# wen-yuan-zhang/Fast-Learning-NeRF

Hardware: AMD Instinct MI355X
Metric: training rays/sec (Lego-like 800x800, 64+128 samples) + PSNR@N-iters (higher is better)
Workload: dtype f32; 1 GPU; nerf-ours Lego full 800x800 (BASELINE configs[1]), SURVEY 8(d) throughput protocol: 4096 uniformly drawn rays per GPU per step, 64+128 samples, use_viewdirs, white_bkgd, perturb=1, U[0,1) targets, random-init nets, leaf-error table on, fp32-width bf16x6 kernels, plain backward (FASTNERF_COMPACT=0); parallelism=dp1, math_mode=bf16x6, backward=plain (every sample)

## Files before the change

fast-learning-nerf_amd/_lib.py:

```python
import ctypes as C
import os

import torch

HERE = os.path.dirname(os.path.abspath(__file__))
LIB_PATH = os.environ.get('FASTNERF_LIB') or os.path.join(HERE, 'libfastnerf.so')

P = C.c_void_p
I = C.c_int
L = C.c_int64
F = C.c_float
D = C.c_double
U64 = C.c_uint64



class StepArgs(C.Structure):
    _fields_ = (
        [('n', L)] + [(k, P) for k in ('rays_o', 'rays_d', 'target', 't_rand', 'u', 'noise0', 'noise1')]
        + [('seed0', U64), ('seed1', U64), ('leaf_tag', P), ('table', P), ('net_floats', L)]
        + [(k, P) for k in ('params', 'grads', 'adam_m', 'adam_v', 'packed_fwd_c', 'packed_bwd_c', 'packed_fwd_f', 'packed_bwd_f',
                            'rays11', 'z0', 'raw0', 'act0', 'rgb0', 'disp0', 'acc0', 'w0', 'depth0',
                            'z1', 'z_samples', 'z_std', 'raw1', 'act1', 'rgb1', 'disp1', 'acc1', 'w1', 'depth1',
                            'g_rgb', 'g_rgb0', 'loss2', 'draw_ws', 'act_ws', 'dact_ws', 'partial_ws', 'live_ws', 'counts')]
        + [(k, D) for k in ('focal', 'lr', 'beta1', 'beta2', 'eps')]
        + [(k, F) for k in ('near_plane', 'far_plane', 'grad_scale')]
        + [(k, I) for k in ('math_mode', 'N_samples', 'N_importance', 'lindisp', 'perturb', 'white_bkgd', 'ndc', 'H', 'W', 'live',
                            'fwd_flags', 'max_leaves', 'adam_t')]
        + [('occ', P), ('occ_counts', P)])


class OccGrid(C.Structure):
    _fields_ = [('words', P), ('lo', F * 3), ('inv', F * 3), ('n', C.c_int32 * 3), ('outside_occupied', C.c_int32)]


OCC_MAX_LEVELS = 8


class OccCascade(C.Structure):
    _fields_ = [('levels', C.c_int32), ('reserved', C.c_int32), ('level', OccGrid * OCC_MAX_LEVELS)]


STEP_FORWARD, STEP_BWD_FINE, STEP_BWD_COARSE, STEP_UPDATE = 1, 2, 4, 8

SIGNATURES = {
    'fastnerf_version': (I, []),
    'fastnerf_last_error': (C.c_char_p, []),
    'fastnerf_device_cus': (I, []),
    'fastnerf_gen_rays': (I, [I, I, F, F, F, F, P, P, P, P]),
    'fastnerf_gen_rays_pixels': (I, [L, P, P, F, F, F, F, P, P, P]),
    'fastnerf_ndc_rays': (I, [L, I, I, D, F, P, P, P, P, P]),
    'fastnerf_pack_rays': (I, [L, P, P, F, F, I, I, I, D, P, P]),
    'fastnerf_sample_coarse': (I, [L, I, P, I, I, P, U64, P, P]),
    'fastnerf_posenc': (I, [L, I, P, P, P]),
    'fastnerf_mlp_pack': (I, [P, P, P, P]),
    'fastnerf_mlp_fwd': (I, [L, I, P, P, P, P, P, P, P]),
    'fastnerf_mlp_bwd_partial_floats': (L, []),
    'fastnerf_mlp_bwd': (I, [L, I, P, P, P, P, P, P, P, P]),
    'fastnerf_raw2outputs_fwd': (I, [L, I, P, P, P, P, I, P, P, P, P, P, P]),
    'fastnerf_raw2outputs_bwd': (I, [L, I, P, P, P, P, I, P, P, P]),
    'fastnerf_raw2outputs_bwd_full': (I, [L, I, P, P, P, P, I, P, P, P, P, P, P, P, P, P]),
    'fastnerf_sample_pdf_merge': (I, [L, I, I, P, P, I, P, U64, P, P, P, P]),
    'fastnerf_sample_pdf': (I, [L, I, I, P, P, I, P, U64, P, P]),
    'fastnerf_mse_leafmax': (I, [L, P, P, P, F, P, P, P, P, I, P, P]),
    'fastnerf_adam_step': (I, [L, P, P, P, P, D, D, D, D, I, P]),
    'fastnerf_net_floats': (L, [I, I]),
    'fastnerf_mlp_act_floats': (L, [I, L]),
    'fastnerf_mlp_pack_ex': (I, [I, P, P, P, P]),
    'fastnerf_mlp_fwd_ex': (I, [I, L, I, P, P, P, P, P, P, P]),
    'fastnerf_mlp_bwd_ex': (I, [I, L, I, P, P, P, P, P, P, P, P]),
    'fastnerf_mlp_bf16_floats': (L, [I, I, L]),
    'fastnerf_mlp_bf16_partial_floats': (L, []),
    'fastnerf_mlp_bf16_pack': (I, [I, P, P, P, P]),
    'fastnerf_mlp_bf16_fwd': (I, [I, L, I, P, P, P, P, P, P, P]),
    'fastnerf_mlp_bf16_bwd': (I, [I, L, I, P, P, P, P, P, P, P, P]),
    'fastnerf_render_rays_fwd': (I, [I, L, I, I, P, I, I, I, I, P, P, P, P, U64, U64, P, P, P, P] + [P] * 18 + [P]),
    'fastnerf_render_rays_fwd_ex': (I, [I, L, I, I, P, I, I, I, I, P, P, P, P, U64, U64, P, P, P, P] + [P] * 18 + [I, P]),
    'fastnerf_mlp_bf16_fwd_flags': (I, [I, L, I, P, P, P, P, P, I, P]),
    'fastnerf_mlp_fwd_flags_ex': (I, [I, L, I, P, P, P, P, P, I, P]),
    'fastnerf_render_rays_bwd': (I, [I, L, I, I, P, I] + [P] * 20),
    'fastnerf_pp_intersect_sphere': (I, [L, P, P, P, P]),
    'fastnerf_pp_fg_depths': (I, [L, I, F, P, I, P, U64, P, P]),
    'fastnerf_pp_sample_pdf_merge': (I, [L, I, I, P, P, I, P, U64, P, P, P]),
    'fastnerf_pp_perturb_samples': (I, [L, I, P, P, U64, P, P]),
    'fastnerf_pp_sample_pdf': (I, [L, I, I, P, P, I, P, U64, P, P]),
    'fastnerf_pp_depth2pts_outside': (I, [L, I, P, P, P, P, P, P]),
    'fastnerf_pp_composite_fwd': (I, [L, I, I, P, P, P, P, P, P, P, P, P]),
    'fastnerf_pp_composite_bwd': (I, [L, I, I, P, P, P, P, P, P, P, P]),
    'fastnerf_pp_gen_rays': (I, [I, I, P, P, P, P, P]),
    'fastnerf_leaf_sumcount': (I, [L, P, P, P, I, P, P, P]),
    'fastnerf_tree_adjust_mean': (L, [P, P, P, I, D]),
    'fastnerf_tree_create': (P, [I, I, I, I]),
    'fastnerf_tree_destroy': (None, [P]),
    'fastnerf_tree_num_leaves': (I, [P, I]),
    'fastnerf_tree_max_leaves': (I, [P]),
    'fastnerf_tree_min_area': (D, [P, I]),
    'fastnerf_tree_get_leaves': (I, [P, I, P]),
    'fastnerf_tree_set_leaves': (I, [P, I, I, P, D]),
    'fastnerf_tree_leaf_plan': (I, [P, I, D, I, P]),
    'fastnerf_tree_adjust': (L, [P, P, I, D]),
    'fastnerf_tree_epoch_plan': (L, [P, D, I, P, P]),
# ... 99 lines not shown
```

fast-learning-nerf_amd/csrc/mlp_bwd_dw.hip:

```cpp
#include "mlp_common.h"

int fn_launch_dx(int mm, int grid, hipStream_t st, int64_t P, const float* draw, const float* act, const float* params, const float* packed_bwd,
                 float* dact, const NetLayout& L, const int* live_idx, const int* live_cnt);

#define DW_MT 32

template <int WO, int WI, int TO, int TI, bool BIAS, bool RANK1>
__global__ void __launch_bounds__(WO * WI * 64, WO * WI / 4)
mlp_bwd_dw_kernel(int64_t P, const float* __restrict__ dY, int ldy, const float* __restrict__ X, int ldx,
                  const float* __restrict__ draw , float* __restrict__ partial_w,
                  float* __restrict__ partial_b, float* __restrict__ partial_r, const int* __restrict__ live_idx,
                  const int* __restrict__ live_cnt) {
  if (live_idx) P = (int64_t)__builtin_amdgcn_readfirstlane(*live_cnt);
  constexpr int NO = WO * TO * 32, KI = WI * TI * 32;
  constexpr int NTD = WO * WI * 64;
  constexpr int STAGE = DW_MT * (NO + KI) + DW_MT;
  extern __shared__ __attribute__((aligned(16))) float smem[];
  const int tid = threadIdx.x;
  const int lane = tid & 63;
  const int wave = __builtin_amdgcn_readfirstlane(tid >> 6);
  const int wo = wave / WI, wi = wave % WI;
  const int64_t ntile_all = (P + DW_MT - 1) / DW_MT;
  const int64_t per = (ntile_all + gridDim.x - 1) / gridDim.x;
  const int64_t t0 = blockIdx.x * per;
  int64_t t1 = t0 + per;
  if (t1 > ntile_all) t1 = ntile_all;

  f32x16 acc[TO][TI];
#pragma unroll
  for (int a = 0; a < TO; ++a)
#pragma unroll
    for (int b = 0; b < TI; ++b)
#pragma unroll
      for (int r = 0; r < 16; ++r) acc[a][b][r] = 0.f;
  float bsum = 0.f, rsum = 0.f;

  constexpr int YV = (DW_MT * NO / 4 + NTD - 1) / NTD;
  constexpr int XV = (DW_MT * KI / 4 + NTD - 1) / NTD;
  static_assert(DW_MT * NO % 4 == 0 && DW_MT * KI % 4 == 0 && NO <= NTD && KI <= NTD, "stage split");
  float4 ry[YV], rx[XV];
  float rda = 0.f;

  auto load_stage = [&](int64_t t) {
    const int64_t pbase = t * DW_MT;
#pragma unroll
    for (int i = 0; i < YV; ++i) {
      const int e = (i * NTD + tid) * 4;
      const int m = e / NO, c = e % NO;
      const int64_t p = pbase + m;
      ry[i] = (e < DW_MT * NO && p < P) ? *reinterpret_cast<const float4*>(dY + p * ldy + c)
                                        : make_float4(0.f, 0.f, 0.f, 0.f);
    }
#pragma unroll
// ... 294 lines not shown
    const int nwhole = (relmax + 1) / 16;
    int dmain = nwhole >= 5 ? (nwhole - 3) / 2 : 0;
    if (dmain > n2) dmain = n2;
#pragma unroll 1
    for (int d = 0; d < dmain; ++d) pair(d, WHOLE);
#pragma unroll 1
    for (int d = dmain; d < n2; ++d) pair(d, ANY);
  }
  float* pw = partial_w + (int64_t)wg * NO * KI;
#pragma unroll
  for (int i = 0; i < TO; ++i)
#pragma unroll
    for (int j = 0; j < TI; ++j)
#pragma unroll
      for (int r = 0; r < 16; ++r) {
        const int o = (wo * TO + i) * 32 + crow(r, lane);
        const int c = (wi * TI + j) * 32 + (lane & 31);
        pw[(int64_t)o * KI + c] = acc[i][j][r];
      }
  if (BIAS || RANK1) {
#pragma unroll
    for (int k = 0; k < TPW; ++k) {
      const int t = k * NW + wave;
      if (NTILE % NW == 0 || t < NTILE) {
        const float sv = ssum[k] + __shfl_xor(ssum[k], 32, 64);
        if (lane < 32) {
          if (BIAS && t < CTO1) partial_b[(int64_t)wg * NO1 + t * 32 + lane] = sv;
          if (RANK1 && t >= CTO && t < CTO + CTI1) partial_r[(int64_t)wg * KI1 + (t - CTO) * 32 + lane] = sv;
        }
      }
    }
  }
}

template <int WO, int WI, int TO, int TI, bool BIAS, bool RANK1, int CTI2 = 0, int CTO2 = 0>
__global__ void __launch_bounds__(WO * WI * 64, WO * WI / 4)
mlp_bwd_dw6_kernel(int64_t P, const float* __restrict__ dY, const float* __restrict__ X,
                   const float* __restrict__ draw, float* __restrict__ partial_w, float* __restrict__ partial_b,
                   float* __restrict__ partial_r, const int* __restrict__ live_idx, const int* __restrict__ live_cnt,
                   const float* __restrict__ X2 = nullptr, const float* __restrict__ dY2 = nullptr) {
  if (live_idx) P = (int64_t)__builtin_amdgcn_readfirstlane(*live_cnt);
  dw6_body<WO, WI, TO, TI, BIAS, RANK1, CTI2, CTO2>(P, dY, X, draw, partial_w, partial_b, partial_r, live_idx, X2, dY2, (int)blockIdx.x,
                                                    (int)gridDim.x);
}

#define DW_QMAX 256
__host__ __device__ static inline int dw_trunk_chunks(int64_t P, int ncu) {
  const int unit = ncu >= 8 ? ncu / 8 : 1;
  const int64_t nq = (P + 15) / 16;
  int64_t k = (nq + (int64_t)unit * DW_QMAX - 1) / ((int64_t)unit * DW_QMAX);
  k = k < 1 ? 1 : (k > 8 ? 8 : k);
  return unit * (int)k;
}
#define DW_TRUNK_JOBS 7
struct DwTrunk {
  const float* dY[DW_TRUNK_JOBS];
  const float* X[DW_TRUNK_JOBS];
  float* pw[DW_TRUNK_JOBS];
  float* pb[DW_TRUNK_JOBS];
};
__global__ void __launch_bounds__(512, 2)
mlp_bwd_dw6_trunk_kernel(int64_t P, DwTrunk J, const int* __restrict__ live_idx, const int* __restrict__ live_cnt, int ncu) {
  if (live_idx) P = (int64_t)__builtin_amdgcn_readfirstlane(*live_cnt);
  const int nact = dw_trunk_chunks(P, ncu);
  if ((int)blockIdx.x >= nact) return;
  const int job = (int)blockIdx.y;
  dw6_body<4, 2, 2, 4, true, false>(P, J.dY[job], J.X[job], nullptr, J.pw[job], J.pb[job], nullptr, live_idx, nullptr, nullptr,
                                    (int)blockIdx.x, nact);
}

__global__ void __launch_bounds__(128) head_grads_kernel(int64_t P, const float* __restrict__ draw,
                                                          const float* __restrict__ hv,
                                                          float* __restrict__ partial, const int* __restrict__ live_idx,
                                                          const int* __restrict__ live_cnt) {
  const int k = threadIdx.x;
  if (live_idx) P = *live_cnt;
  auto dptr = [&](int64_t q) { return draw + (live_idx ? (int64_t)live_idx[q] : q) * 4; };
  const int64_t per = (P + gridDim.x - 1) / gridDim.x;
  const int64_t pa = blockIdx.x * per;
  int64_t pb = pa + per;
  if (pb > P) pb = P;
  float s0 = 0.f, s1 = 0.f, s2 = 0.f, sb = 0.f;
  int64_t p = pa;
  constexpr int NF = 16;
  for (; p + NF <= pb; p += NF) {
    float4 d[NF];
    float h[NF];
#pragma unroll
    for (int i = 0; i < NF; ++i) {
      d[i] = *reinterpret_cast<const float4*>(dptr(p + i));
      h[i] = hv[(p + i) * 128 + k];
    }
#pragma unroll
    for (int i = 0; i < NF; ++i) {
      s0 = fmaf(d[i].x, h[i], s0); s1 = fmaf(d[i].y, h[i], s1); s2 = fmaf(d[i].z, h[i], s2);
      if (k < 4) sb += (k == 0) ? d[i].x : (k == 1) ? d[i].y : (k == 2) ? d[i].z : d[i].w;
    }
  }
  for (; p < pb; ++p) {
    const float4 d = *reinterpret_cast<const float4*>(dptr(p));
    const float h = hv[p * 128 + k];
    s0 = fmaf(d.x, h, s0); s1 = fmaf(d.y, h, s1); s2 = fmaf(d.z, h, s2);
    if (k < 4) sb += (k == 0) ? d.x : (k == 1) ? d.y : (k == 2) ? d.z : d.w;
  }
  float* o = partial + (int64_t)blockIdx.x * 388;
  o[k] = s0; o[128 + k] = s1; o[256 + k] = s2;
  if (k < 4) o[384 + k] = sb;
}

struct RedSeg {
  int64_t src;
  int64_t wg_stride;
  int64_t dst;
  int nwg, rows, cols, ld, valid_cols;
  int dyn;
  int sc_cols;
  int64_t sc_dst;
};
#define MAX_SEGS 32
struct RedTable {
  RedSeg s[MAX_SEGS];
  int n;
};

__global__ void __launch_bounds__(256) reduce_all_kernel(RedTable tab, const float* __restrict__ partial, float* __restrict__ grads,
                                                          float* __restrict__ scratch, int64_t P, const int* __restrict__ live_cnt, int ncu) {
  RedSeg sg = tab.s[blockIdx.y];
  if (sg.dyn) {
    if (live_cnt) P = (int64_t)*live_cnt;
    const int n = dw_trunk_chunks(P, ncu);
    sg.nwg = n < sg.nwg ? n : sg.nwg;
  }
  const int64_t total = (int64_t)sg.rows * sg.cols;
  const float* src = partial + sg.src;
  for (int64_t e = blockIdx.x * (int64_t)blockDim.x + threadIdx.x; e < total; e += (int64_t)gridDim.x * blockDim.x) {
    const int r = (int)(e / sg.cols), c = (int)(e % sg.cols);
    if (c >= sg.valid_cols) continue;
    constexpr int RS = 16;
    float a[RS];
#pragma unroll
    for (int i = 0; i < RS; ++i) a[i] = 0.f;
    int w = 0;
    for (; w + RS <= sg.nwg; w += RS) {
#pragma unroll
      for (int i = 0; i < RS; ++i) a[i] += src[(int64_t)(w + i) * sg.wg_stride + e];
    }
#pragma unroll
    for (int i = 0; i < RS - 1; ++i)
      if (w + i < sg.nwg) a[i] += src[(int64_t)(w + i) * sg.wg_stride + e];
#pragma unroll
    for (int h = RS / 2; h >= 1; h >>= 1)
#pragma unroll
      for (int i = 0; i < h; ++i) a[i] += a[i + h];
    if (c < sg.sc_cols) scratch[sg.sc_dst + (int64_t)r * sg.sc_cols + c] = a[0];
    else grads[sg.dst + (int64_t)r * sg.ld + c] = a[0];
  }
}

__global__ void __launch_bounds__(256) unfold_kernel(const float* __restrict__ G, const float* __restrict__ params, float* __restrict__ grads,
                                                      int64_t VW, int64_t VB, int64_t FW, int64_t FB) {
  __shared__ double As[16][17], Bs[16][17];
  const int tx = threadIdx.x & 15, ty = threadIdx.x >> 4;
  const int b = blockIdx.x;
  if (b == 384) {
    const int i = threadIdx.x;
    double s = 0.0;
    for (int o = 0; o < 128; ++o) s = fma((double)params[VW + (int64_t)o * 283 + i], (double)grads[VB + o], s);
    grads[FB + i] = (float)s;
    return;
  }
  const bool wf = b < 256;
  const int r0 = wf ? (b >> 4) * 16 : ((b - 256) >> 4) * 16, c0 = (b & 15) * 16;
  const int K = wf ? 128 : 256;
  double s = 0.0;
  for (int k0 = 0; k0 < K; k0 += 16) {
    if (wf) {
// ... 37 lines not shown
  }
  return o;
}
extern "C" int64_t fastnerf_mlp_bwd_partial_floats(void) {
  return dw_job_base(12, num_cus(), 96) + (int64_t)HEAD_MAX_WG * 388;
}

template <int WO, int WI, int TO, int TI, bool BIAS, bool RANK1, int MM = MM_F32, int CTI2 = 0, int CTO2 = 0>
static int launch_dw(int64_t P, const float* dY, int ldy, const float* X, int ldx, const float* draw, float* base,
                     int nwg, hipStream_t st, const int* live_idx = nullptr, const int* live_cnt = nullptr,
                     const float* X2 = nullptr, const float* dY2 = nullptr, float* pr_at = nullptr) {
  constexpr int NO = WO * TO * 32, KI = WI * TI * 32;
  float* pw = base;
  float* pb = base + (int64_t)nwg * NO * KI;
  float* pr = pr_at ? pr_at : pb + (BIAS ? (int64_t)nwg * (NO - CTO2 * 32) : 0);
  if constexpr (MM == MM_X6) {
    if (ldy != NO - CTO2 * 32 || ldx != KI - CTI2 * 32 || (CTI2 > 0) != (X2 != nullptr) || (CTO2 > 0) != (dY2 != nullptr)) {
      fn::set_error("launch_dw: the bf16x6 dW kernel needs ld == width (and X2 / dY2 exactly when CTI2 / CTO2 > 0)");
      return -1;
    }
    constexpr int lds6 = 2 * (WO * TO + WI * TI) * 3 * 1024 + 128;
    auto kern6 = mlp_bwd_dw6_kernel<WO, WI, TO, TI, BIAS, RANK1, CTI2, CTO2>;
    static bool attr6 = false;
    if (!attr6) {
      FN_HIP(hipFuncSetAttribute(reinterpret_cast<const void*>(kern6), hipFuncAttributeMaxDynamicSharedMemorySize, lds6));
      attr6 = true;
    }
    hipLaunchKernelGGL(kern6, dim3(nwg), dim3(WO * WI * 64), lds6, st, P, dY, X, draw, pw, pb, pr, live_idx, live_cnt, X2, dY2);
    FN_LAUNCH_CHECK();
    return 0;
  } else {
    static_assert(MM == MM_F32 && CTI2 == 0 && CTO2 == 0, "two-tensor jobs exist for the bf16x6 dW kernel only");
    constexpr int STAGE = DW_MT * (NO + KI) + DW_MT;
    const size_t lds = 2 * STAGE * sizeof(float);
    auto kern = mlp_bwd_dw_kernel<WO, WI, TO, TI, BIAS, RANK1>;
    static bool attr = false;
    if (!attr) {
      FN_HIP(hipFuncSetAttribute(reinterpret_cast<const void*>(kern), hipFuncAttributeMaxDynamicSharedMemorySize, (int)lds));
      attr = true;
    }
    hipLaunchKernelGGL(kern, dim3(nwg), dim3(WO * WI * 64), lds, st, P, dY, ldy, X, ldx, draw, pw, pb, pr, live_idx, live_cnt);
    FN_LAUNCH_CHECK();
    return 0;
  }
}

static void add_seg(RedTable& T, int64_t src, int64_t wg_stride, int nwg, int rows, int cols, int64_t dst, int ld,
                    int valid_cols, int dyn = 0, int sc_cols = 0, int64_t sc_dst = 0) {
  RedSeg& s = T.s[T.n++];
  s.src = src; s.wg_stride = wg_stride; s.nwg = nwg; s.rows = rows; s.cols = cols; s.dst = dst; s.ld = ld;
  s.valid_cols = valid_cols; s.dyn = dyn; s.sc_cols = sc_cols; s.sc_dst = sc_dst;
}

template <int MM>
static int bwd_launch_t(int kind, int64_t n, int S, const float* draw, const float* act, const float* params,
                      const float* packed_bwd, float* dact, float* partial, float* grads, const int* live_idx,
                      const int* live_cnt, fn_stream_t stream) {
  constexpr int MW = MM;
  const NetLayout& L = layout_of(kind);
  const int PEP = L.pe_pad;
  hipStream_t st = fn::S(stream);
  const int64_t P = n * S;
  const int64_t ntiles = (P + TM - 1) / TM;
  const int ncu = num_cus();
  int grid = ncu * WG_PER_CU;
  if (ntiles < grid) grid = (int)ntiles;
  if (int rc_dx = fn_launch_dx(MM, grid, st, P, draw, act, params, packed_bwd, dact, L, live_idx, live_cnt)) return rc_dx;

  const int nwg = ncu;
  RedTable T;
  T.n = 0;
  int rc;
  const float* a_pe = act + act_pe(P, PEP);
  auto region = [&](int j) { return partial + dw_job_base(j, ncu, PEP); };
  auto segs = [&](int j, int64_t dstW, int ld, int validc, int64_t dstB, int64_t dstR, int dyn = 0) {
    const DwJobDesc d = dw_job(j, PEP);
    const int64_t b = dw_job_base(j, ncu, PEP);
    add_seg(T, b, (int64_t)d.NO * d.KI, nwg, d.NO, d.KI, dstW, ld, validc, dyn);
    int64_t o = b + (int64_t)nwg * d.NO * d.KI;
    if (d.bias) { add_seg(T, o, d.NO, nwg, 1, d.NO, dstB, d.NO, d.NO, dyn); o += (int64_t)nwg * d.NO; }
    if (d.rank1) add_seg(T, o, d.KI, nwg, 1, d.KI, dstR, d.KI, d.KI, dyn);
  };
  if constexpr (MW == MM_X6) {
    if (PEP == 64) rc = launch_dw<8, 2, 2, 1, true, false, MW, 0, 8>(P, dact + dact_y(P, 0), 256, a_pe, 64, nullptr, region(0), nwg, st, live_idx, live_cnt, nullptr, dact + dact_y(P, 5));
    else rc = launch_dw<8, 1, 2, 3, true, false, MW, 0, 8>(P, dact + dact_y(P, 0), 256, a_pe, 96, nullptr, region(0), nwg, st, live_idx, live_cnt, nullptr, dact + dact_y(P, 5));
    if (rc) return rc;
    const int64_t b0 = dw_job_base(0, ncu, PEP);
    add_seg(T, b0, (int64_t)512 * PEP, nwg, 256, PEP, L.LW[0], L.in_pe, L.in_pe);
    add_seg(T, b0 + (int64_t)256 * PEP, (int64_t)512 * PEP, nwg, 256, PEP, L.LW[5], 256 + L.in_pe, L.in_pe);
    add_seg(T, b0 + (int64_t)nwg * 512 * PEP, 256, nwg, 1, 256, L.LB[0], 256, 256);
  } else {
    if (PEP == 64) rc = launch_dw<4, 1, 2, 2, true, false, MW>(P, dact + dact_y(P, 0), 256, a_pe, 64, nullptr, region(0), nwg, st, live_idx, live_cnt);
    else rc = launch_dw<4, 1, 2, 3, true, false, MW>(P, dact + dact_y(P, 0), 256, a_pe, 96, nullptr, region(0), nwg, st, live_idx, live_cnt);
    if (rc) return rc;
    segs(0, L.LW[0], L.in_pe, L.in_pe, L.LB[0], 0);
  }
  if constexpr (MW != MM_X6) {
    for (int l = 1; l < 8; ++l) {
      if ((rc = launch_dw<4, 2, 2, 4, true, false, MW>(P, dact + dact_y(P, l), 256, act + act_h(P, PEP, l - 1), 256, nullptr, region(l), nwg, st, live_idx, live_cnt))) return rc;
      segs(l, L.LW[l] + (l == 5 ? L.in_pe : 0), l == 5 ? 256 + L.in_pe : 256, 256, L.LB[l], 0);
    }
  }
  if constexpr (MW != MM_X6) {
    if (PEP == 64) rc = launch_dw<4, 1, 2, 2, false, false, MW>(P, dact + dact_y(P, 5), 256, a_pe, 64, nullptr, region(8), nwg, st, live_idx, live_cnt);
    else rc = launch_dw<4, 1, 2, 3, false, false, MW>(P, dact + dact_y(P, 5), 256, a_pe, 96, nullptr, region(8), nwg, st, live_idx, live_cnt);
    if (rc) return rc;
    segs(8, L.LW[5], 256 + L.in_pe, L.in_pe, 0, 0);
  }
  if constexpr (MW == MM_X6) {
    DwTrunk J;
    for (int l = 1; l < 8; ++l) {
      J.dY[l - 1] = dact + dact_y(P, l);
      J.X[l - 1] = act + act_h(P, PEP, l - 1);
      J.pw[l - 1] = region(l);
      J.pb[l - 1] = region(l) + (int64_t)nwg * 256 * 256;
    }
    constexpr int lds6 = 2 * 16 * 3 * 1024 + 128;
    static bool attr_t = false;
    if (!attr_t) {
      FN_HIP(hipFuncSetAttribute(reinterpret_cast<const void*>(mlp_bwd_dw6_trunk_kernel), hipFuncAttributeMaxDynamicSharedMemorySize, lds6));
      attr_t = true;
    }
    hipLaunchKernelGGL(mlp_bwd_dw6_trunk_kernel, dim3(dw_trunk_chunks(P, ncu), DW_TRUNK_JOBS), dim3(512), lds6, st, P, J, live_idx, live_cnt, ncu);
    FN_LAUNCH_CHECK();
    for (int l = 1; l < 8; ++l) segs(l, L.LW[l] + (l == 5 ? L.in_pe : 0), l == 5 ? 256 + L.in_pe : 256, 256, L.LB[l], 0, 1);
  }
  float* const pr_view = region(9);
  const int64_t g_off = dw_job_base(9, ncu, PEP) + (int64_t)nwg * 256;
  if constexpr (MW == MM_X6) {
    if ((rc = launch_dw<4, 3, 1, 3, true, true, MW, 1, 0>(P, dact + dact_yv(P), 128, act + act_h(P, PEP, 7), 256, draw, region(10), nwg, st,
                                                    live_idx, live_cnt, act + act_vpe(P, PEP), nullptr, pr_view))) return rc;
    const int64_t b10 = dw_job_base(10, ncu, PEP);
    add_seg(T, b10, 128 * 288, nwg, 128, 288, L.VW, 283, 283, 0, 256, g_off);
    add_seg(T, b10 + (int64_t)nwg * 128 * 288, 128, nwg, 1, 128, L.VB, 128, 128);
  } else {
    if ((rc = launch_dw<2, 4, 2, 2, true, true, MW>(P, dact + dact_yv(P), 128, act + act_h(P, PEP, 7), 256, draw, region(10), nwg, st, live_idx, live_cnt,
                                              nullptr, nullptr, pr_view))) return rc;
    const int64_t b10 = dw_job_base(10, ncu, PEP);
    add_seg(T, b10, 128 * 256, nwg, 128, 256, L.VW, 283, 256, 0, 256, g_off);
    add_seg(T, b10 + (int64_t)nwg * 128 * 256, 128, nwg, 1, 128, L.VB, 128, 128);
    if ((rc = launch_dw<4, 1, 1, 1, false, false, MW>(P, dact + dact_yv(P), 128, act + act_vpe(P, PEP), 32, nullptr, region(11), nwg, st, live_idx, live_cnt))) return rc;
    segs(11, L.VW + 256, 283, 27, 0, 0);
  }
  add_seg(T, dw_job_base(9, ncu, PEP), 256, nwg, 1, 256, L.AW, 256, 256);
  {
    const int hg = HEAD_MAX_WG;
    const int64_t hb = dw_job_base(12, ncu, PEP);
    hipLaunchKernelGGL(head_grads_kernel, dim3(hg), dim3(128), 0, st, P, draw, act + act_hv(P, PEP), partial + hb, live_idx, live_cnt);
    FN_LAUNCH_CHECK();
    add_seg(T, hb, 388, hg, 1, 388, L.RW, 388, 387);
    add_seg(T, hb + 387, 388, hg, 1, 1, L.AB, 1, 1);
  }
  hipLaunchKernelGGL(reduce_all_kernel, dim3(256, T.n), dim3(256), 0, st, T, partial, grads, partial, P, live_cnt, ncu);
  FN_LAUNCH_CHECK();
  hipLaunchKernelGGL(unfold_kernel, dim3(385), dim3(256), 0, st, partial + g_off, params, grads, L.VW, L.VB, L.FW, L.FB);
  FN_LAUNCH_CHECK();
  return 0;
}
static int bwd_launch(int kind, int64_t n, int S, const float* draw, const float* act, const float* params,
                      const float* packed_bwd, float* dact, float* partial, float* grads, const int* live_idx,
                      const int* live_cnt, fn_stream_t stream, int mm = MM_F32) {
  return mm == MM_X6 ? bwd_launch_t<MM_X6>(kind, n, S, draw, act, params, packed_bwd, dact, partial, grads, live_idx, live_cnt, stream)
                     : bwd_launch_t<MM_F32>(kind, n, S, draw, act, params, packed_bwd, dact, partial, grads, live_idx, live_cnt, stream);
}
extern "C" int fastnerf_mlp_bwd_ex(int kind, int64_t n, int S, const float* draw, const float* act,
                                   const float* params, const float* packed_bwd, float* dact, float* partial,
                                   float* grads, fn_stream_t stream) {
  FN_CHECK_ARG(kind >= 0 && kind <= 2 && n > 0 && S >= 1, "kind in 0..2, n>0, S>=1");
  FN_CHECK_ARG(draw && act && params && packed_bwd && dact && partial && grads, "null pointer");
  return bwd_launch(kind, n, S, draw, act, params, packed_bwd, dact, partial, grads, nullptr, nullptr, stream);
}
extern "C" int fastnerf_mlp_bwd_live_ex(int kind, int64_t n, int S, const float* draw, const float* act,
                                        const float* params, const float* packed_bwd, float* dact, float* partial,
                                        float* grads, const int32_t* live_idx, const int32_t* live_cnt,
                                        fn_stream_t stream) {
  FN_CHECK_ARG(kind >= 0 && kind <= 2 && n > 0 && S >= 1, "kind in 0..2, n>0, S>=1");
  FN_CHECK_ARG(draw && act && params && packed_bwd && dact && partial && grads && live_idx && live_cnt, "null pointer");
  return bwd_launch(kind, n, S, draw, act, params, packed_bwd, dact, partial, grads, live_idx, live_cnt, stream);
}
extern "C" int fastnerf_mlp_bwd(int64_t n, int S, const float* draw, const float* act, const float* params,
                                const float* packed_bwd, float* dact, float* partial, float* grads,
                                fn_stream_t stream) {
  return fastnerf_mlp_bwd_ex(0, n, S, draw, act, params, packed_bwd, dact, partial, grads, stream);
}

extern "C" int fastnerf_mlp_x6_bwd(int kind, int64_t n, int S, const float* draw, const float* act, const float* params,
                                   const float* packed_bwd, float* dact, float* partial, float* grads, fn_stream_t stream) {
  FN_CHECK_ARG(kind >= 0 && kind <= 2 && n > 0 && S >= 1, "kind in 0..2, n>0, S>=1");
  FN_CHECK_ARG(draw && act && params && packed_bwd && dact && partial && grads, "null pointer");
  return bwd_launch(kind, n, S, draw, act, params, packed_bwd, dact, partial, grads, nullptr, nullptr, stream, MM_X6);
}
extern "C" int fastnerf_mlp_x6_bwd_live(int kind, int64_t n, int S, const float* draw, const float* act, const float* params,
                                        const float* packed_bwd, float* dact, float* partial, float* grads,
                                        const int32_t* live_idx, const int32_t* live_cnt, fn_stream_t stream) {
  FN_CHECK_ARG(kind >= 0 && kind <= 2 && n > 0 && S >= 1, "kind in 0..2, n>0, S>=1");
  FN_CHECK_ARG(draw && act && params && packed_bwd && dact && partial && grads && live_idx && live_cnt, "null pointer");
  return bwd_launch(kind, n, S, draw, act, params, packed_bwd, dact, partial, grads, live_idx, live_cnt, stream, MM_X6);
}
```

fast-learning-nerf_amd/csrc/render.cpp:

```cpp
#include <stdint.h>
#include "../../include/fastnerf.h"

namespace fn {
void set_error(const char* fmt, ...);
const char* occ_cascade_fault(const fn_occ_cascade* c);
}

struct MlpMode {
  int (*pack)(int kind, const float* params, float* packed_fwd, float* packed_bwd, fn_stream_t);
  int (*fwd)(int kind, int64_t n, int S, const float* rays11, const float* z, const float* params, const float* packed_fwd, float* raw,
             float* act, int flags, fn_stream_t);
  int (*fwd_list)(int kind, int64_t n, int S, const float* rays11, const float* z, const float* params, const float* packed_fwd,
                  float* raw, const int32_t* live_idx, const int32_t* live_cnt, int flags, fn_stream_t);
  int (*fwd_live)(int kind, int64_t n, int S, const float* rays11, const float* z, const float* params, const float* packed_fwd,
                  float* act, const int32_t* live_idx, const int32_t* live_cnt, fn_stream_t);
  int (*bwd)(int kind, int64_t n, int S, const float* draw, const float* act, const float* params, const float* packed_bwd, float* dact,
             float* partial, float* grads, fn_stream_t);
  int (*bwd_live)(int kind, int64_t n, int S, const float* draw, const float* act, const float* params, const float* packed_bwd,
                  float* dact, float* partial, float* grads, const int32_t* live_idx, const int32_t* live_cnt, fn_stream_t);
};

static int fwd_fp32(int kind, int64_t n, int S, const float* rays11, const float* z, const float* params, const float* packed_fwd,
                    float* raw, float* act, int flags, fn_stream_t stream) {
  return act ? fastnerf_mlp_fwd_ex(kind, n, S, rays11, z, params, packed_fwd, raw, act, stream)
             : fastnerf_mlp_fwd_flags_ex(kind, n, S, rays11, z, params, packed_fwd, raw, flags, stream);
}

static int fwd_bf16(int kind, int64_t n, int S, const float* rays11, const float* z, const float* params, const float* packed_fwd,
                    float* raw, float* act, int flags, fn_stream_t stream) {
  return act ? fastnerf_mlp_bf16_fwd(kind, n, S, rays11, z, params, packed_fwd, raw, act, stream)
             : fastnerf_mlp_bf16_fwd_flags(kind, n, S, rays11, z, params, packed_fwd, raw, flags, stream);
}

static const MlpMode modes[3] = {
    {fastnerf_mlp_pack_ex, fwd_fp32, fastnerf_mlp_fwd_list_ex, fastnerf_mlp_fwd_live_ex, fastnerf_mlp_bwd_ex, fastnerf_mlp_bwd_live_ex},
    {fastnerf_mlp_bf16_pack, fwd_bf16, fastnerf_mlp_bf16_fwd_list, fastnerf_mlp_bf16_fwd_live, fastnerf_mlp_bf16_bwd,
     fastnerf_mlp_bf16_bwd_live},
    {fastnerf_mlp_x6_pack, fastnerf_mlp_x6_fwd, fastnerf_mlp_x6_fwd_list, fastnerf_mlp_x6_fwd_live, fastnerf_mlp_x6_bwd,
     fastnerf_mlp_x6_bwd_live},
};

struct RrFwd {
  const char* fname;
  int math_mode;
  int64_t n;
  int N_samples, N_importance;
  const float* rays11;
  int lindisp, perturb, det, white_bkgd;
  const float *t_rand, *u, *noise0, *noise1;
  uint64_t seed0, seed1;
  const float *params_c, *packed_c, *params_f, *packed_f;
  float *z0, *raw0, *rgb0, *disp0, *acc0, *w0, *depth0, *z1, *z_samples, *z_std, *raw1, *rgb1, *disp1, *acc1, *w1, *depth1;
  int flags;
  fn_stream_t stream;
};

static bool rr_fwd_scalars(const RrFwd& a) {
  if (a.math_mode < 0 || a.math_mode > 2 || a.n < 0 || a.N_samples < 2 || a.N_importance < 0) {
// ... 101 lines not shown
                                                    int lindisp, int perturb, int det, int white_bkgd, const float* t_rand,
                                                    const float* u, uint64_t seed0, uint64_t seed1, const float* params_c,
                                                    const float* packed_c, const float* params_f, const float* packed_f,
                                                    const fn_occ_cascade* cascade, int32_t* live_ws, int32_t* counts_out, float* z0,
                                                    float* raw0, float* rgb0, float* disp0, float* acc0, float* w0, float* depth0,
                                                    float* z1, float* z_samples, float* z_std, float* raw1, float* rgb1, float* disp1,
                                                    float* acc1, float* w1, float* depth1, int flags, fn_stream_t stream) {
  return rr_fwd_occ({"fastnerf_render_rays_fwd_occ_cascade", math_mode, n, N_samples, N_importance, rays11, lindisp, perturb, det,
                     white_bkgd, t_rand, u, nullptr, nullptr, seed0, seed1, params_c, packed_c, params_f, packed_f, z0, raw0, rgb0,
                     disp0, acc0, w0, depth0, z1, z_samples, z_std, raw1, rgb1, disp1, acc1, w1, depth1, flags, stream},
                    nullptr, cascade, live_ws, counts_out);
}

extern "C" int fastnerf_render_rays_fwd(int math_mode, int64_t n, int N_samples, int N_importance, const float* rays11,
                                        int lindisp, int perturb, int det, int white_bkgd, const float* t_rand, const float* u,
                                        const float* noise0, const float* noise1, uint64_t seed0, uint64_t seed1,
                                        const float* params_c, const float* packed_c, const float* params_f,
                                        const float* packed_f, float* z0, float* raw0, float* act0, float* rgb0,
                                        float* disp0, float* acc0, float* w0, float* depth0, float* z1,
                                        float* z_samples, float* z_std, float* raw1, float* act1, float* rgb1,
                                        float* disp1, float* acc1, float* w1, float* depth1, fn_stream_t stream) {
  return fastnerf_render_rays_fwd_ex(math_mode, n, N_samples, N_importance, rays11, lindisp, perturb, det, white_bkgd, t_rand, u,
                                     noise0, noise1, seed0, seed1, params_c, packed_c, params_f, packed_f, z0, raw0, act0, rgb0,
                                     disp0, acc0, w0, depth0, z1, z_samples, z_std, raw1, act1, rgb1, disp1, acc1, w1, depth1, 0,
                                     stream);
}

static int rr_bwd(int math_mode, int64_t n, int N_samples, int N_importance, const float* rays11,
                  int white_bkgd, const float* g_rgb, const float* g_rgb0, const float* noise0,
                  const float* noise1, const float* z0, const float* raw0, const float* act0,
                  const float* z1, const float* raw1, const float* act1, const float* params_c,
                  const float* packed_bwd_c, const float* params_f, const float* packed_bwd_f,
                  float* draw_ws, float* dact_ws, float* partial_ws, float* grads_c, float* grads_f,
                  int passes, fn_stream_t stream) {
  if (math_mode < 0 || math_mode > 2 || n <= 0 || N_samples < 2 || N_importance < 0) {
    fn::set_error("fastnerf_render_rays_bwd: bad argument: math_mode in {0,1,2}, n>0, N_samples>=2, N_importance>=0");
    return -1;
  }
  if (!rays11 || !z0 || !raw0 || !act0 || !params_c || !packed_bwd_c || !draw_ws || !dact_ws || !partial_ws || !grads_c) {
    fn::set_error("fastnerf_render_rays_bwd: null pointer (coarse pass)");
    return -1;
  }
  int rc;
  auto mlp = [&](int S, const float* act, const float* params, const float* packed, float* grads) {
    return modes[math_mode].bwd(0, n, S, draw_ws, act, params, packed, dact_ws, partial_ws, grads, stream);
  };
  const float* g_coarse = g_rgb;
  if (N_importance > 0) {
    if (!g_rgb || !g_rgb0 || !z1 || !raw1 || !act1 || !params_f || !packed_bwd_f || !grads_f) {
      fn::set_error("fastnerf_render_rays_bwd: null pointer (fine pass)");
      return -1;
    }
    const int S1 = N_samples + N_importance;
    if (passes & 1) {
      if ((rc = fastnerf_raw2outputs_bwd(n, S1, raw1, z1, rays11, noise1, white_bkgd, g_rgb, draw_ws, stream))) return rc;
      if ((rc = mlp(S1, act1, params_f, packed_bwd_f, grads_f))) return rc;
    }
    g_coarse = g_rgb0;
  }
  if (!g_coarse) {
    fn::set_error("fastnerf_render_rays_bwd: null gradient");
    return -1;
  }
  if (!(passes & 2)) return 0;
  if ((rc = fastnerf_raw2outputs_bwd(n, N_samples, raw0, z0, rays11, noise0, white_bkgd, g_coarse, draw_ws, stream))) return rc;
  return mlp(N_samples, act0, params_c, packed_bwd_c, grads_c);
}

extern "C" int fastnerf_render_rays_bwd(int math_mode, int64_t n, int N_samples, int N_importance, const float* rays11,
                                        int white_bkgd, const float* g_rgb, const float* g_rgb0, const float* noise0,
                                        const float* noise1, const float* z0, const float* raw0, const float* act0,
                                        const float* z1, const float* raw1, const float* act1, const float* params_c,
                                        const float* packed_bwd_c, const float* params_f, const float* packed_bwd_f,
                                        float* draw_ws, float* dact_ws, float* partial_ws, float* grads_c, float* grads_f,
                                        fn_stream_t stream) {
  return rr_bwd(math_mode, n, N_samples, N_importance, rays11, white_bkgd, g_rgb, g_rgb0, noise0, noise1, z0, raw0, act0, z1, raw1,
                act1, params_c, packed_bwd_c, params_f, packed_bwd_f, draw_ws, dact_ws, partial_ws, grads_c, grads_f, 3, stream);
}


static int rr_bwd_live(int math_mode, int64_t n, int N_samples, int N_importance, const float* rays11, int white_bkgd,
                       const float* g_rgb, const float* g_rgb0, const float* noise0, const float* noise1,
                       const float* z0, const float* raw0, const float* z1, const float* raw1,
                       const float* params_c, const float* packed_fwd_c, const float* packed_bwd_c,
                       const float* params_f, const float* packed_fwd_f, const float* packed_bwd_f,
                       float* draw_ws, float* act_ws, float* dact_ws, float* partial_ws, int32_t* live_ws,
                       float* grads_c, float* grads_f, int32_t* counts_out, int passes, fn_stream_t stream) {
  if (math_mode < 0 || math_mode > 2 || n <= 0 || N_samples < 2 || N_importance < 0) {
    fn::set_error("fastnerf_render_rays_bwd_live: bad argument: math_mode in {0,1,2}, n>0, N_samples>=2, N_importance>=0");
    return -1;
  }
  if (!rays11 || !z0 || !raw0 || !params_c || !packed_fwd_c || !packed_bwd_c || !draw_ws || !act_ws || !dact_ws ||
      !partial_ws || !live_ws || !grads_c) {
    fn::set_error("fastnerf_render_rays_bwd_live: null pointer (coarse pass)");
    return -1;
  }
  const int S1 = N_samples + N_importance;
  int32_t* cnt = live_ws;
  int32_t* idx = live_ws + 4;
  int32_t* cws = idx + n * (int64_t)S1;
  int rc;
  auto pass = [&](int S, const float* z, const float* raw, const float* noise, const float* g, const float* params,
                  const float* pf, const float* pb, float* grads, int32_t* cnt_out) -> int {
    if ((rc = fastnerf_raw2outputs_bwd(n, S, raw, z, rays11, noise, white_bkgd, g, draw_ws, stream))) return rc;
    if ((rc = fastnerf_compact_live(n * (int64_t)S, draw_ws, idx, cnt_out, cws, stream))) return rc;
    if ((rc = modes[math_mode].fwd_live(0, n, S, rays11, z, params, pf, act_ws, idx, cnt_out, stream))) return rc;
// ... 123 lines not shown
```

include/fastnerf.h:

```cpp
#ifndef FASTNERF_H
#define FASTNERF_H
#include <stdint.h>
#ifdef __cplusplus
extern "C" {
#endif

typedef void* fn_stream_t;

int fastnerf_version(void);
const char* fastnerf_last_error(void);
int fastnerf_device_cus(void);

int fastnerf_gen_rays(int H, int W, float fx, float fy, float cx, float cy, const float* c2w_host,
                      float* rays_o, float* rays_d, fn_stream_t stream);
int fastnerf_gen_rays_pixels(int64_t n, const int32_t* pix, const float* poses, float fx, float fy, float cx,
                             float cy, float* rays_o, float* rays_d, fn_stream_t stream);
int fastnerf_ndc_rays(int64_t n, int H, int W, double focal, float near, const float* rays_o, const float* rays_d,
                      float* out_o, float* out_d, fn_stream_t stream);
int fastnerf_pack_rays(int64_t n, const float* rays_o, const float* rays_d, float near, float far, int ndc, int H,
                       int W, double focal, float* rays11, fn_stream_t stream);
int fastnerf_sample_coarse(int64_t n, int S, const float* rays11, int lindisp, int perturb, const float* t_rand,
                           uint64_t seed, float* z, fn_stream_t stream);
int fastnerf_posenc(int64_t n, int L, const float* x, float* out, fn_stream_t stream);

#define FASTNERF_NET_PARAMS 595844
#define FASTNERF_PACKED_FWD 593920
#define FASTNERF_PACKED_BWD 557056
#define FASTNERF_ACT_FLOATS 2592
#define FASTNERF_ACT_SLACK 8192
#define FASTNERF_DACT_FLOATS 2432

int fastnerf_mlp_pack(const float* params, float* packed_fwd, float* packed_bwd, fn_stream_t stream);
int fastnerf_mlp_fwd(int64_t n, int S, const float* rays11, const float* z, const float* params,
                     const float* packed_fwd, float* raw, float* act, fn_stream_t stream);
int64_t fastnerf_mlp_bwd_partial_floats(void);
int fastnerf_mlp_bwd(int64_t n, int S, const float* draw, const float* act, const float* params,
                     const float* packed_bwd, float* dact, float* partial, float* grads, fn_stream_t stream);

int fastnerf_raw2outputs_fwd(int64_t n, int S, const float* raw, const float* z, const float* rays11,
                             const float* noise, int white_bkgd, float* rgb_map, float* disp, float* acc,
                             float* weights, float* depth, fn_stream_t stream);
int fastnerf_raw2outputs_bwd(int64_t n, int S, const float* raw, const float* z, const float* rays11,
                             const float* noise, int white_bkgd, const float* g_rgb, float* draw,
                             fn_stream_t stream);
int fastnerf_raw2outputs_bwd_full(int64_t n, int S, const float* raw, const float* z, const float* rays11,
                                  const float* noise, int white_bkgd, const float* acc, const float* depth,
                                  const float* g_rgb, const float* g_disp, const float* g_acc, const float* g_w,
                                  const float* g_depth, float* draw, fn_stream_t stream);
int fastnerf_sample_pdf_merge(int64_t n, int S, int Ni, const float* z, const float* weights, int det,
                              const float* u, uint64_t seed, float* z_out, float* z_samples, float* z_std,
                              fn_stream_t stream);

int fastnerf_sample_pdf(int64_t n, int M, int Ni, const float* bins, const float* weights, int det, const float* u,
                        uint64_t seed, float* samples, fn_stream_t stream);

int fastnerf_mse_leafmax(int64_t n, const float* rgb, const float* rgb0, const float* target, float grad_scale,
                         float* g_rgb, float* g_rgb0, float* loss2, const int32_t* leaf_tag, int max_leaves,
                         uint32_t* table, fn_stream_t stream);
int fastnerf_adam_step(int64_t n, float* params, const float* grads, float* m, float* v, double lr, double beta1,
                       double beta2, double eps, int step, fn_stream_t stream);

int64_t fastnerf_net_floats(int kind, int what);
int64_t fastnerf_mlp_act_floats(int kind, int64_t n_points);
int fastnerf_mlp_pack_ex(int kind, const float* params, float* packed_fwd, float* packed_bwd, fn_stream_t stream);
// ... 252 lines not shown
```

Baseline: 245,500 rays/s.

## Merge fine and coarse bf16x6 trunk weight-gradient passes into one paired launch

In bf16x6 mode with both passes requested, the fine and coarse backward passes now defer their trunk weight-gradient kernel and reductions. A single paired kernel then covers both networks' trunk jobs in one grid, followed by the two reductions. The coarse pass runs on a separately allocated side workspace (dact and partial buffers), so the two passes do not overwrite each other. This is meant to fill the GPU better, since each trunk launch alone may underuse the CUs, and to remove a launch boundary. In exchange it costs extra device memory and a lazy hipMalloc, and it falls back to the old path when allocation fails or during graph capture.

```diff
diff --git a/fast-learning-nerf_amd/_lib.py b/fast-learning-nerf_amd/_lib.py
--- a/fast-learning-nerf_amd/_lib.py
+++ b/fast-learning-nerf_amd/_lib.py
@@ -47,6 +47,7 @@
     'fastnerf_version': (I, []),
     'fastnerf_last_error': (C.c_char_p, []),
     'fastnerf_device_cus': (I, []),
+    'fastnerf_x6_pair_launches': (L, []),
     'fastnerf_gen_rays': (I, [I, I, F, F, F, F, P, P, P, P]),
     'fastnerf_gen_rays_pixels': (I, [L, P, P, F, F, F, F, P, P, P]),
     'fastnerf_ndc_rays': (I, [L, I, I, D, F, P, P, P, P, P]),
diff --git a/fast-learning-nerf_amd/csrc/dw_pair.h b/fast-learning-nerf_amd/csrc/dw_pair.h
--- /dev/null
+++ b/fast-learning-nerf_amd/csrc/dw_pair.h
@@ -0,0 +1,34 @@
+#pragma once
+#include <stdint.h>
+
+#define DW_TRUNK_JOBS 7
+struct DwTrunk {
+  const float* dY[DW_TRUNK_JOBS];
+  const float* X[DW_TRUNK_JOBS];
+  float* pw[DW_TRUNK_JOBS];
+  float* pb[DW_TRUNK_JOBS];
+};
+
+struct RedSeg {
+  int64_t src;
+  int64_t wg_stride;
+  int64_t dst;
+  int nwg, rows, cols, ld, valid_cols;
+  int dyn;
+  int sc_cols;
+  int64_t sc_dst;
+};
+#define MAX_SEGS 32
+struct RedTable {
+  RedSeg s[MAX_SEGS];
+  int n;
+};
+
+struct DwDeferred {
+  DwTrunk J;
+  RedTable T;
+  int64_t P, g_off;
+  const float* params;
+  float *partial, *grads;
+  int kind;
+};
diff --git a/fast-learning-nerf_amd/csrc/mlp_bwd_dw.hip b/fast-learning-nerf_amd/csrc/mlp_bwd_dw.hip
--- a/fast-learning-nerf_amd/csrc/mlp_bwd_dw.hip
+++ b/fast-learning-nerf_amd/csrc/mlp_bwd_dw.hip
@@ -1,4 +1,8 @@
 #include "mlp_common.h"
+#include "dw_pair.h"
+#include <atomic>
+#include <map>
+#include <utility>
 
 int fn_launch_dx(int mm, int grid, hipStream_t st, int64_t P, const float* draw, const float* act, const float* params, const float* packed_bwd,
                  float* dact, const NetLayout& L, const int* live_idx, const int* live_cnt);
@@ -399,13 +403,6 @@
   k = k < 1 ? 1 : (k > 8 ? 8 : k);
   return unit * (int)k;
 }
-#define DW_TRUNK_JOBS 7
-struct DwTrunk {
-  const float* dY[DW_TRUNK_JOBS];
-  const float* X[DW_TRUNK_JOBS];
-  float* pw[DW_TRUNK_JOBS];
-  float* pb[DW_TRUNK_JOBS];
-};
 __global__ void __launch_bounds__(512, 2)
 mlp_bwd_dw6_trunk_kernel(int64_t P, DwTrunk J, const int* __restrict__ live_idx, const int* __restrict__ live_cnt, int ncu) {
   if (live_idx) P = (int64_t)__builtin_amdgcn_readfirstlane(*live_cnt);
@@ -414,6 +411,25 @@
   const int job = (int)blockIdx.y;
   dw6_body<4, 2, 2, 4, true, false>(P, J.dY[job], J.X[job], nullptr, J.pw[job], J.pb[job], nullptr, live_idx, nullptr, nullptr,
                                     (int)blockIdx.x, nact);
+}
+
+struct DwTrunkPair {
+  DwTrunk J[2];
+  int64_t P[2];
+};
+__global__ void __launch_bounds__(512, 2)
+mlp_bwd_dw6_trunk_pair_kernel(DwTrunkPair A, int ncu) {
+  const int c0 = dw_trunk_chunks(A.P[0], ncu);
+  int b = (int)blockIdx.x;
+  const int pass = b >= DW_TRUNK_JOBS * c0 ? 1 : 0;
+  if (pass) b -= DW_TRUNK_JOBS * c0;
+  const int64_t P = A.P[pass];
+  const int nact = pass ? dw_trunk_chunks(P, ncu) : c0;
+  const int job = b / nact;
+  if (job >= DW_TRUNK_JOBS) return;
+  const DwTrunk& J = A.J[pass];
+  dw6_body<4, 2, 2, 4, true, false>(P, J.dY[job], J.X[job], nullptr, J.pw[job], J.pb[job], nullptr, nullptr, nullptr, nullptr, b - job * nact,
+                                    nact);
 }
 
 __global__ void __launch_bounds__(128) head_grads_kernel(int64_t P, const float* __restrict__ draw,
@@ -455,20 +471,6 @@
   if (k < 4) o[384 + k] = sb;
 }
 
-struct RedSeg {
-  int64_t src;
-  int64_t wg_stride;
-  int64_t dst;
-  int nwg, rows, cols, ld, valid_cols;
-  int dyn;
-  int sc_cols;
-  int64_t sc_dst;
-};
-#define MAX_SEGS 32
-struct RedTable {
-  RedSeg s[MAX_SEGS];
-  int n;
-};
 
 __global__ void __launch_bounds__(256) reduce_all_kernel(RedTable tab, const float* __restrict__ partial, float* __restrict__ grads,
                                                           float* __restrict__ scratch, int64_t P, const int* __restrict__ live_cnt, int ncu) {
@@ -612,10 +614,40 @@
   s.valid_cols = valid_cols; s.dyn = dyn; s.sc_cols = sc_cols; s.sc_dst = sc_dst;
 }
 
+#define FN_MAX_DEV 64
+template <class K>
+static int trunk_lds_attr(K kern, bool (&done)[FN_MAX_DEV], int lds) {
+  int dev = 0;
+  FN_HIP(hipGetDevice(&dev));
+  if (dev < 0 || dev >= FN_MAX_DEV || !done[dev]) {
+    FN_HIP(hipFuncSetAttribute(reinterpret_cast<const void*>(kern), hipFuncAttributeMaxDynamicSharedMemorySize, lds));
+    if (dev >= 0 && dev < FN_MAX_DEV) done[dev] = true;
+  }
+  return 0;
+}
+constexpr int DW_TRUNK_LDS = 2 * 16 * 3 * 1024 + 128;
+static int trunk_chunks_fit(int64_t P, int ncu, int nwg) {
+  if (dw_trunk_chunks(P, ncu) > nwg) {
+    fn::set_error("mlp_bwd: the trunk launch needs %d chunks per job, the partial regions hold %d (a device with fewer than 8 CUs?)",
+                  dw_trunk_chunks(P, ncu), nwg);
+    return -1;
+  }
+  return 0;
+}
+
+static int bwd_reduce(const RedTable& T, const NetLayout& L, int64_t P, const float* params, float* partial, float* grads, int64_t g_off,
+                      const int* live_cnt, int ncu, hipStream_t st) {
+  hipLaunchKernelGGL(reduce_all_kernel, dim3(256, T.n), dim3(256), 0, st, T, partial, grads, partial, P, live_cnt, ncu);
+  FN_LAUNCH_CHECK();
+  hipLaunchKernelGGL(unfold_kernel, dim3(385), dim3(256), 0, st, partial + g_off, params, grads, L.VW, L.VB, L.FW, L.FB);
+  FN_LAUNCH_CHECK();
+  return 0;
+}
+
 template <int MM>
 static int bwd_launch_t(int kind, int64_t n, int S, const float* draw, const float* act, const float* params,
                       const float* packed_bwd, float* dact, float* partial, float* grads, const int* live_idx,
-                      const int* live_cnt, fn_stream_t stream) {
+                      const int* live_cnt, fn_stream_t stream, DwDeferred* defer = nullptr) {
   constexpr int MW = MM;
   const NetLayout& L = layout_of(kind);
   const int PEP = L.pe_pad;
@@ -675,14 +707,15 @@
       J.pw[l - 1] = region(l);
       J.pb[l - 1] = region(l) + (int64_t)nwg * 256 * 256;
     }
-    constexpr int lds6 = 2 * 16 * 3 * 1024 + 128;
-    static bool attr_t = false;
-    if (!attr_t) {
-      FN_HIP(hipFuncSetAttribute(reinterpret_cast<const void*>(mlp_bwd_dw6_trunk_kernel), hipFuncAttributeMaxDynamicSharedMemorySize, lds6));
-      attr_t = true;
-    }
-    hipLaunchKernelGGL(mlp_bwd_dw6_trunk_kernel, dim3(dw_trunk_chunks(P, ncu), DW_TRUNK_JOBS), dim3(512), lds6, st, P, J, live_idx, live_cnt, ncu);
-    FN_LAUNCH_CHECK();
+    if ((rc = trunk_chunks_fit(P, ncu, nwg))) return rc;
+    if (defer) {
+      defer->J = J;
+    } else {
+      static bool attr_t[FN_MAX_DEV] = {};
+      if ((rc = trunk_lds_attr(mlp_bwd_dw6_trunk_kernel, attr_t, DW_TRUNK_LDS))) return rc;
+      hipLaunchKernelGGL(mlp_bwd_dw6_trunk_kernel, dim3(dw_trunk_chunks(P, ncu), DW_TRUNK_JOBS), dim3(512), DW_TRUNK_LDS, st, P, J, live_idx, live_cnt, ncu);
+      FN_LAUNCH_CHECK();
+    }
     for (int l = 1; l < 8; ++l) segs(l, L.LW[l] + (l == 5 ? L.in_pe : 0), l == 5 ? 256 + L.in_pe : 256, 256, L.LB[l], 0, 1);
   }
   float* const pr_view = region(9);
@@ -711,12 +744,95 @@
     add_seg(T, hb, 388, hg, 1, 388, L.RW, 388, 387);
     add_seg(T, hb + 387, 388, hg, 1, 1, L.AB, 1, 1);
   }
-  hipLaunchKernelGGL(reduce_all_kernel, dim3(256, T.n), dim3(256), 0, st, T, partial, grads, partial, P, live_cnt, ncu);
+  if (defer) {
+    defer->T = T; defer->P = P; defer->g_off = g_off; defer->params = params; defer->partial = partial; defer->grads = grads; defer->kind = kind;
+    return 0;
+  }
+  return bwd_reduce(T, L, P, params, partial, grads, g_off, live_cnt, ncu, st);
+}
+
+namespace fn {
+struct PairWs {
+  float *dact = nullptr, *partial = nullptr;
+  int64_t dact_cap = 0, partial_cap = 0;
+  int64_t refused = 0;
+};
+static std::mutex g_pair_mu;
+static std::map<std::pair<int, hipStream_t>, PairWs> g_pair;
+static std::atomic<int64_t> g_pair_launches{0};
+
+static bool pair_grow(PairWs& w, float*& p, int64_t& cap, int64_t need) {
+  if (cap >= need) return true;
+  if (w.refused > 0 && need >= w.refused) return false;
+  hipStreamCaptureMode mode = hipStreamCaptureModeRelaxed;
+  (void)hipThreadExchangeStreamCaptureMode(&mode);
+  if (p) (void)hipFree(p);
+  p = nullptr;
+  cap = 0;
+  const bool ok = hipMalloc(reinterpret_cast<void**>(&p), sizeof(float) * (size_t)need) == hipSuccess;
+  (void)hipThreadExchangeStreamCaptureMode(&mode);
+  if (!ok) {
+    (void)hipGetLastError();
+    p = nullptr;
+    w.refused = need;
+    fprintf(stderr, "fastnerf: no memory for the side workspace of the paired bf16x6 backward (%.2f GB): this stream keeps the per-pass trunk launches\n",
+            4e-9 * (double)need);
+    return false;
+  }
+  cap = need;
+  return true;
+}
+
+bool x6_pair_workspace(int64_t P_coarse, fn_stream_t stream, float** dact2, float** partial2) {
+  hipStream_t st = S(stream);
+  hipStreamCaptureStatus cs = hipStreamCaptureStatusNone;
+  if (hipStreamIsCapturing(st, &cs) != hipSuccess) {
+    (void)hipGetLastError();
+    return false;
+  }
+  if (cs != hipStreamCaptureStatusNone) return false;
+  int dev = 0;
+  if (hipGetDevice(&dev) != hipSuccess) return false;
+  std::lock_guard<std::mutex> lk(g_pair_mu);
+  PairWs& w = g_pair[{dev, st}];
+  if (!pair_grow(w, w.dact, w.dact_cap, P_coarse * (int64_t)DACT_FLOATS) ||
+      !pair_grow(w, w.partial, w.partial_cap, fastnerf_mlp_bwd_partial_floats()))
+    return false;
+  *dact2 = w.dact;
+  *partial2 = w.partial;
+  return true;
+}
+
+int x6_pair_pass(DwDeferred* d, int64_t n, int S, const float* draw, const float* act, const float* params, const float* packed_bwd,
+                 float* dact, float* partial, float* grads, fn_stream_t stream) {
+  FN_CHECK_ARG(d && n > 0 && S >= 1, "d != NULL, n>0, S>=1");
+  FN_CHECK_ARG(draw && act && params && packed_bwd && dact && partial && grads, "null pointer");
+  return bwd_launch_t<MM_X6>(0, n, S, draw, act, params, packed_bwd, dact, partial, grads, nullptr, nullptr, stream, d);
+}
+
+int x6_pair_finish(const DwDeferred* fine, const DwDeferred* coarse, fn_stream_t stream) {
+  hipStream_t st = S(stream);
+  const int ncu = num_cus();
+  const DwDeferred* d[2] = {fine, coarse};
+  DwTrunkPair A;
+  int nwg = 0;
+  for (int k = 0; k < 2; ++k) {
+    A.J[k] = d[k]->J;
+    A.P[k] = d[k]->P;
+    nwg += DW_TRUNK_JOBS * dw_trunk_chunks(A.P[k], ncu);
+  }
+  static bool attr_p[FN_MAX_DEV] = {};
+  if (int rc = trunk_lds_attr(mlp_bwd_dw6_trunk_pair_kernel, attr_p, DW_TRUNK_LDS)) return rc;
+  hipLaunchKernelGGL(mlp_bwd_dw6_trunk_pair_kernel, dim3(nwg), dim3(512), DW_TRUNK_LDS, st, A, ncu);
   FN_LAUNCH_CHECK();
-  hipLaunchKernelGGL(unfold_kernel, dim3(385), dim3(256), 0, st, partial + g_off, params, grads, L.VW, L.VB, L.FW, L.FB);
-  FN_LAUNCH_CHECK();
+  g_pair_launches.fetch_add(1, std::memory_order_relaxed);
+  for (int k = 0; k < 2; ++k)
+    if (int rc = bwd_reduce(d[k]->T, layout_of(d[k]->kind), d[k]->P, d[k]->params, d[k]->partial, d[k]->grads, d[k]->g_off, nullptr, ncu, st)) return rc;
   return 0;
 }
+}
+extern "C" int64_t fastnerf_x6_pair_launches(void) { return fn::g_pair_launches.load(std::memory_order_relaxed); }
+
 static int bwd_launch(int kind, int64_t n, int S, const float* draw, const float* act, const float* params,
                       const float* packed_bwd, float* dact, float* partial, float* grads, const int* live_idx,
                       const int* live_cnt, fn_stream_t stream, int mm = MM_F32) {
diff --git a/fast-learning-nerf_amd/csrc/render.cpp b/fast-learning-nerf_amd/csrc/render.cpp
--- a/fast-learning-nerf_amd/csrc/render.cpp
+++ b/fast-learning-nerf_amd/csrc/render.cpp
@@ -1,9 +1,14 @@
 #include <stdint.h>
 #include "../../include/fastnerf.h"
+#include "dw_pair.h"
 
 namespace fn {
 void set_error(const char* fmt, ...);
 const char* occ_cascade_fault(const fn_occ_cascade* c);
+bool x6_pair_workspace(int64_t P_coarse, fn_stream_t stream, float** dact2, float** partial2);
+int x6_pair_pass(DwDeferred* d, int64_t n, int S, const float* draw, const float* act, const float* params, const float* packed_bwd,
+                 float* dact, float* partial, float* grads, fn_stream_t stream);
+int x6_pair_finish(const DwDeferred* fine, const DwDeferred* coarse, fn_stream_t stream);
 }
 
 struct MlpMode {
@@ -211,6 +216,15 @@
       return -1;
     }
     const int S1 = N_samples + N_importance;
+    float *dact2 = nullptr, *partial2 = nullptr;
+    if (passes == 3 && math_mode == 2 && fn::x6_pair_workspace(n * (int64_t)N_samples, stream, &dact2, &partial2)) {
+      DwDeferred d_fine, d_coarse;
+      if ((rc = fastnerf_raw2outputs_bwd(n, S1, raw1, z1, rays11, noise1, white_bkgd, g_rgb, draw_ws, stream))) return rc;
+      if ((rc = fn::x6_pair_pass(&d_fine, n, S1, draw_ws, act1, params_f, packed_bwd_f, dact_ws, partial_ws, grads_f, stream))) return rc;
+      if ((rc = fastnerf_raw2outputs_bwd(n, N_samples, raw0, z0, rays11, noise0, white_bkgd, g_rgb0, draw_ws, stream))) return rc;
+      if ((rc = fn::x6_pair_pass(&d_coarse, n, N_samples, draw_ws, act0, params_c, packed_bwd_c, dact2, partial2, grads_c, stream))) return rc;
+      return fn::x6_pair_finish(&d_fine, &d_coarse, stream);
+    }
     if (passes & 1) {
       if ((rc = fastnerf_raw2outputs_bwd(n, S1, raw1, z1, rays11, noise1, white_bkgd, g_rgb, draw_ws, stream))) return rc;
       if ((rc = mlp(S1, act1, params_f, packed_bwd_f, grads_f))) return rc;
diff --git a/include/fastnerf.h b/include/fastnerf.h
--- a/include/fastnerf.h
+++ b/include/fastnerf.h
@@ -10,6 +10,7 @@
 int fastnerf_version(void);
 const char* fastnerf_last_error(void);
 int fastnerf_device_cus(void);
+int64_t fastnerf_x6_pair_launches(void);
 
 int fastnerf_gen_rays(int H, int W, float fx, float fy, float cx, float cy, const float* c2w_host,
                       float* rays_o, float* rays_d, fn_stream_t stream);
```

Result: faster. 251,800 rays/s, median of 6 (+2.6%).
